# tj12323/GeoPurify

Measured on AMD Instinct MI355X. Metric: scenes/sec (ScanNet-val shape) + pooled-feature GB/s vs HBM peak, higher is better.
Workload: dtype f32 (student convolutions and pooling: f16 hi/lo split operands, 3 MFMAs per product, fp32 accumulate)

## Files before the change

### geopurify_amd/_lib.py

```python
import ctypes
import os
from ctypes import POINTER, c_char_p, c_double, c_float, c_int32, c_int64, c_size_t, c_uint32, c_uint64, c_void_p

_HERE = os.path.dirname(os.path.abspath(__file__))
LIB_PATH = os.environ.get("GP_LIB") or os.path.join(_HERE, "libgeopurify_hip.so")

_P = c_void_p
GP_KNN_MAX_K = 127
GP_KNN_QUERY_MAX_K = 32
GP_ELEM_F32, GP_ELEM_F16, GP_ELEM_BF16 = 0, 1, 2
GP_LABEL_U8, GP_LABEL_I16, GP_LABEL_I32, GP_LABEL_I64 = 0, 1, 2, 3

SIGNATURES = {
    "gp_version": (c_int32, []),
    "gp_last_error": (c_char_p, []),
    "gp_debug_set": (c_int32, [c_int32, c_int32]),
    "gp_debug_ptr": (c_int32, [c_int32, _P, c_size_t]),
    "gp_voxelize_workspace_bytes": (c_size_t, [c_int64]),
    "gp_voxelize_f64": (c_int32, [_P, c_int64, POINTER(c_double), _P, _P, _P, _P, _P, _P, _P, c_size_t, _P]),
    "gp_fnv_hash_f64": (c_int32, [_P, c_int64, _P, _P]),
    "gp_project_points_f64": (c_int32, [_P, c_int64, POINTER(c_double), c_double, c_double, c_double,
                                        c_double, _P, c_int32, c_int32, c_int32, c_double, _P, _P, _P]),
    "gp_render_depth_f64": (c_int32, [_P, c_int64, POINTER(c_double), c_double, c_double, c_double, c_double,
                                      c_int32, c_int32, c_int32, _P, _P]),
# ... 51 lines not shown
    "gp_pool_tiles_workspace_bytes": (c_size_t, [c_int64, c_int32]),
    "gp_pool_tiles_count": (c_int32, [_P, c_int64, c_int32, c_int32, _P, _P, c_size_t, _P]),
    "gp_pool_tiles_fill": (c_int32, [_P, _P, c_int64, c_int32, c_int32, _P, _P, _P, _P]),
    "gp_pool_tiles_apply": (c_int32, [_P, c_int64, _P, _P, _P, c_int32, c_int64, c_int32, _P, c_int64, _P]),
    "gp_pool_mfma_workspace_bytes": (c_size_t, [c_int64, c_int32]),
    "gp_pool_mfma_count": (c_int32, [_P, c_int64, c_int32, c_int32, c_int32, _P, _P, _P, c_size_t, _P]),
    "gp_pool_mfma_fill": (c_int32, [_P, _P, c_int64, c_int32, c_int32, _P, _P, c_int64, _P, _P, _P, _P]),
    "gp_pool_mfma_apply": (c_int32, [_P, _P, c_int64, _P, _P, _P, _P, c_int64, c_int32, c_int32, _P, _P, c_int64, _P, c_int64, _P, _P]),
    "gp_pool_mfma_apply_persistent": (c_int32, [_P, _P, c_int64, _P, _P, _P, _P, c_int64, c_int32, c_int32, c_int32, _P, _P, c_int64,
                                                _P, c_int64, c_int64, _P, _P, _P]),
    "gp_pool_cs_workspace_bytes": (c_size_t, [c_int64, c_int32]),
    "gp_pool_cs_count": (c_int32, [_P, c_int64, c_int32, c_int32, _P, _P, _P, _P, c_size_t, _P]),
    "gp_pool_cs_fill": (c_int32, [_P, _P, c_int64, c_int32, c_int32, _P, c_int64, c_int32, _P, _P, _P, _P, _P]),
    "gp_pool_cs_structure": (c_int32, [_P, c_int64, c_int32, c_int32, _P, c_int64, c_int32, _P, _P, _P, _P, _P, _P]),
    "gp_pool_cs_structure_valid": (c_int32, [_P, c_int64, c_int32, c_int32, _P, c_int64, c_int32, _P, _P, _P, _P]),
    "gp_affinity_cs_fragments": (c_int32, [_P, _P, c_int64, c_int32, c_int32, c_float, _P, _P, _P, _P, c_int32, _P, _P, _P]),
    "gp_pool_cs_apply": (c_int32, [_P, _P, c_int64, _P, _P, _P, _P, _P, c_int64, c_int32, c_int32, _P, _P, c_int64, _P, c_int64, _P, _P]),
    "gp_pool_cs_deps": (c_int32, [_P, _P, c_int64, c_int32, _P, _P, _P]),
    "gp_pool_cs_chain_flag_words": (c_size_t, [c_int64, c_int32]),
    "gp_pool_cs_chain_flag_words_d": (c_size_t, [c_int64, c_int32, c_int32]),
    "gp_pool_cs_apply_chain": (c_int32, [_P, _P, _P, _P, c_int64, _P, _P, _P, _P, _P, c_int64, c_int32, c_int32, c_int32, _P, c_int64, _P, _P, _P,
                                         c_uint32, _P]),
    "gp_lift_dense_accum": (c_int32, [_P, c_int32, c_int32, c_int32, _P, _P, _P, c_int64, _P, c_int64, _P, _P]),
    "gp_lift_dense_bilinear_accum": (c_int32, [_P, c_int32, c_int32, c_int32, c_int32, c_int32, _P, _P, _P, c_int64, _P,
                                               c_int64, _P, _P]),
    "gp_lift_dense_finish": (c_int32, [_P, c_int64, c_int32, _P, c_int64, _P, _P]),
    "gp_lift_masks_workspace_bytes": (c_size_t, [c_int32, c_int32, c_int32]),
    "gp_lift_masks_view": (c_int32, [_P, c_int32, c_int32, c_int32, _P, _P, _P, _P, _P, c_int32, c_int32,
                                     _P, _P, c_int64, _P, _P, _P, c_size_t, _P]),
    "gp_pv_count": (c_int32, [_P, c_int64, _P, _P]),
# ... 196 lines not shown
```

### geopurify_amd/csrc/pool_mfma_cs.hip

```cpp
#include <cstring>
#include <rocprim/device/device_scan.hpp>

#include "gp_common.h"
#include "gp_gfx950.h"
#include "gp_scan_bytes.h"


namespace {

constexpr int CS_KS = 32;
constexpr int CS_D = 512;
constexpr int CS_DMAX = 1024;
constexpr int CS_BR = 128;
constexpr int CS_NG = CS_BR / 16;
constexpr int CS_NC = 256;
constexpr int CS_NW = 8;
constexpr int CS_WC = CS_NC / CS_NW;
constexpr int CS_MAXID = 16384;
constexpr int CS_MAXNK = 12288;
constexpr int CS_HS = 16384;
constexpr float CS_WSCALE = GP_POOL_CS_WSCALE;

constexpr int CS_RB = CS_NC * 2;
constexpr int CS_PLANE = CS_KS * CS_RB;
// ... 11 lines not shown
}
__device__ __forceinline__ void cs_st_sc1(uint32_t *p, uint32_t v) {
    __hip_atomic_store(p, v, __ATOMIC_RELAXED, __HIP_MEMORY_SCOPE_AGENT);
}
template <typename V>
__device__ __forceinline__ void cs_st16_sc1(void *p, V v) {
    static_assert(sizeof(V) == 16, "16-byte store");
    asm volatile("global_store_dwordx4 %0, %1, off sc1\n\ts_nop 1" ::"v"(p), "v"(v) : "memory");
}

__device__ __forceinline__ void cs_wait_a(f16x8 (&h)[4], f16x8 (&l)[4]) {
    asm volatile("s_waitcnt lgkmcnt(0)"
                 : "+v"(h[0]), "+v"(h[1]), "+v"(h[2]), "+v"(h[3]), "+v"(l[0]), "+v"(l[1]), "+v"(l[2]), "+v"(l[3]));
}

__device__ int cs_union(const int32_t *__restrict__ nbr, int n, int *keys, int *dense, int cap) {
    __shared__ int s_wcnt[16];
    __shared__ int s_base, s_new, s_over;
    const int tid = threadIdx.x, lane = tid & 63, wv = tid >> 6;
    int hs = 2048, shift = 21;
    for (;;) {
        for (int i = tid; i < hs; i += 1024) keys[i] = -1;
        if (tid == 0) { s_base = 0; s_new = 0; s_over = 0; }
        __syncthreads();
        for (int i = tid; i < n; i += 1024) {
            const int id = nbr[i];
            unsigned h = ((unsigned)id * 2654435761u) >> shift;
            int probes = 0;
            while (true) {
                const int old = atomicCAS(&keys[h], -1, id);
                if (old == -1) { atomicAdd(&s_new, 1); break; }
                if (old == id) break;
                h = (h + 1) & (hs - 1);
                if (++probes > (hs < cap ? 256 : hs)) { s_over = 1; break; }
            }
        }
        __syncthreads();
        const bool over = s_over || (hs < cap && s_new > hs / 2);
        __syncthreads();
        if (!over) break;
        if (hs >= cap) return -1;
// ... 1 lines not shown
        shift = 32 - (31 - __clz(cap));
    }
    for (int i0 = 0; i0 < hs; i0 += 1024) {
        const int key = keys[i0 + tid];
        const unsigned long long m = __ballot(key >= 0);
        if (lane == 0) s_wcnt[wv] = __popcll(m);
        __syncthreads();
        int before = s_base;
        for (int w = 0; w < wv; ++w) before += s_wcnt[w];
        if (key >= 0) dense[before + __popcll(m & ((1ull << lane) - 1ull))] = key;
        __syncthreads();
        if (tid == 0) { int tot = 0; for (int w = 0; w < 16; ++w) tot += s_wcnt[w]; s_base += tot; }
        __syncthreads();
    }
    return s_base;
}

__global__ void __launch_bounds__(1024)
cs_count_kernel(const int32_t *__restrict__ nbr, int64_t nv, int k, int rpb, int64_t *__restrict__ padded_cnt, int32_t *__restrict__ bu_n,
                int cap, int second, unsigned long long *__restrict__ stats) {
    extern __shared__ int s_mem[];
    int *keys = s_mem, *dense = s_mem + cap;
    const int64_t b = blockIdx.x, r0 = b * rpb;
    if (second && bu_n[b] >= 0) return;
    const int rows = (int)((nv - r0) < rpb ? (nv - r0) : rpb);
    const int U = cs_union(nbr + r0 * k, rows * k, keys, dense, cap);
    if (threadIdx.x == 0) {
        padded_cnt[b] = U < 0 ? 0 : (int64_t)((U + CS_KS - 1) / CS_KS) * CS_KS;
        bu_n[b] = U;
        if (U > 0 && stats) atomicMax(stats, (unsigned long long)U);
    }
}

constexpr int CS_FILL_WEIGHTS = 0, CS_FILL_DST = 1, CS_FILL_VALID = 2;
template <int MODE>
__global__ void __launch_bounds__(1024)
cs_fill_kernel(const int32_t *__restrict__ nbr, const float *__restrict__ w, int64_t nv, int k, int rpb, const int64_t *__restrict__ bu_off,
               int32_t *__restrict__ bu_row, uint32_t *__restrict__ bu_mask, _Float16 *__restrict__ wa_hi, _Float16 *__restrict__ wa_lo,
               int32_t *__restrict__ dst, uint32_t *__restrict__ valid, int cap) {
    constexpr bool WEIGHTS = MODE == CS_FILL_WEIGHTS;
    extern __shared__ int s_mem[];
    int *A = s_mem, *B = s_mem + cap;
    unsigned short *npos = reinterpret_cast<unsigned short *>(s_mem + 2 * cap);
    const int tid = threadIdx.x;
    const int64_t b = blockIdx.x, r0 = b * rpb;
    const int rows = (int)((nv - r0) < rpb ? (nv - r0) : rpb);
    const int n = rows * k;
    const int32_t *nb = nbr + r0 * k;
    const int U = cs_union(nb, n, A, B, cap);
    int np2 = 1;
    while (np2 < U) np2 <<= 1;
    for (int i = U + tid; i < np2; i += 1024) B[i] = INT32_MAX;
    __syncthreads();
    gp_bitonic_sort_lds(B, np2, tid, 1024);
    for (int i = tid; i < U; i += 1024) A[i] = 0;
    __syncthreads();
    for (int t = tid; t < n; t += 1024) {
        const int id = nb[t];
        int lo = 0, hi = U - 1;
        while (lo < hi) { int mid = (lo + hi) >> 1; if (B[mid] < id) lo = mid + 1; else hi = mid; }
        atomicOr(&A[lo], 1 << ((t / k) >> 4));
    }
    __syncthreads();
    for (int i = tid; i < np2; i += 1024) {
        int key = INT32_MAX;
        if (i < U) {
            const int m = A[i];
            const int first = __ffs(m) - 1, last = 31 - __clz(m);
            key = (first << 28) | (last << 25) | (m << 14) | i;
        }
        A[i] = key;
    }
    __syncthreads();
    gp_bitonic_sort_lds(A, np2, tid, 1024);
    const int64_t o = bu_off[b];
    const int Up = (int)(bu_off[b + 1] - o);
    for (int p = tid; p < Up; p += 1024) {
        const int src = p < U ? (A[p] & 0x3FFF) : (A[0] & 0x3FFF);
        bu_row[o + p] = B[src];
        if (p < U) npos[src] = (unsigned short)p;
    }
    const int64_t ks0 = o / CS_KS;
    __shared__ unsigned s_mask[CS_MAXNK / CS_KS];
    for (int t = tid; t < Up / CS_KS; t += 1024) {
        unsigned m = 0;
        for (int p = t * CS_KS; p < (t + 1) * CS_KS && p < U; ++p) m |= (unsigned)(A[p] >> 14) & 0xFFu;
        bu_mask[ks0 + t] = m;
        s_mask[t] = m;
    }
    __syncthreads();
    if constexpr (MODE == CS_FILL_VALID) {
        const int nsteps = Up / CS_KS;
        const bool in_lds = nsteps * CS_BR <= cap;
        unsigned *sv = reinterpret_cast<unsigned *>(A);
        uint32_t *gv = valid + ks0 * CS_BR;
        __syncthreads();
        for (int i = tid; i < nsteps * CS_BR; i += 1024) { if (in_lds) sv[i] = 0u; else gv[i] = 0u; }
        __syncthreads();
        for (int t = tid; t < n; t += 1024) {
            const int rl = t / k;
            const int id = nb[t];
            int lo = 0, hi = U - 1;
            while (lo < hi) { int mid = (lo + hi) >> 1; if (B[mid] < id) lo = mid + 1; else hi = mid; }
            const int p = npos[lo];
            if (in_lds) atomicOr(&sv[(p / CS_KS) * CS_BR + rl], 1u << (p % CS_KS));
            else atomicOr(&gv[(p / CS_KS) * CS_BR + rl], 1u << (p % CS_KS));
        }
        if (in_lds) {
            __syncthreads();
            for (int i = tid; i < nsteps * CS_BR; i += 1024) gv[i] = sv[i];
        }
        return;
    }
    for (int i = tid; i < (Up / CS_KS) * CS_NG * 64; i += 1024) {
        const int f = i >> 6;
        if ((s_mask[f >> 3] >> (f & 7)) & 1u) {
            const f16x8 z = {0, 0, 0, 0, 0, 0, 0, 0};
            *reinterpret_cast<f16x8 *>(wa_hi + (ks0 * CS_NG * 64 + i) * 8) = z;
            *reinterpret_cast<f16x8 *>(wa_lo + (ks0 * CS_NG * 64 + i) * 8) = z;
        }
    }
    __syncthreads();
    for (int t = tid; t < n; t += 1024) {
        const int rl = t / k;
        const int id = nb[t];
        int lo = 0, hi = U - 1;
        while (lo < hi) { int mid = (lo + hi) >> 1; if (B[mid] < id) lo = mid + 1; else hi = mid; }
        const int p = npos[lo];
        const int64_t ks = ks0 + p / CS_KS;
        const int kk = p % CS_KS;
        const int64_t idx = ((ks * CS_NG + (rl >> 4)) * 64 + (kk >> 3) * 16 + (rl & 15)) * 8 + (kk & 7);
        if constexpr (WEIGHTS) {
            const float v = w[r0 * k + t] * GP_POOL_CS_WSCALE;
            gp_split_f16(v, wa_hi, wa_lo, idx);
        } else {
            dst[r0 * k + t] = (int32_t)idx;
        }
    }
}

struct CsChain {
    const _Float16 *a_hi, *a_lo;
    _Float16 *b_hi, *b_lo;
    int64_t ld;
    uint32_t *flags;
    const int32_t *dep;
    int32_t T;
    uint32_t base;
    int32_t half_sel = -1;
};
constexpr int CS_DEP_CAP = 64;
constexpr int CS_FLAG_HDR = 32;

// ... 738 lines not shown
extern "C" int gp_pool_cs_structure_valid(const int32_t *nbr, int64_t nv, int32_t k, int32_t rows_per_block, const int64_t *bu_off,
                                          int64_t total_rows, int32_t max_union, int32_t *bu_row, uint32_t *bu_mask, uint32_t *bu_valid,
                                          void *stream_) {
    GP_CHECK_ARG(nbr && bu_off && bu_row && bu_mask && bu_valid && nv > 0 && total_rows > 0 && total_rows % CS_KS == 0,
                 "gp_pool_cs_structure_valid: bad argument");
    GP_CHECK_ARG(cs_rpb_ok(rows_per_block), "gp_pool_cs_structure_valid: rows_per_block=%d (16..%d)", rows_per_block, CS_BR);
    GP_CHECK_ARG((int64_t)CS_BR * k <= CS_MAXNK, "gp_pool_cs_structure_valid: k=%d too large (128*k <= %d)", k, CS_MAXNK);
    int64_t nb = (nv + rows_per_block - 1) / rows_per_block;
    hipStream_t s = gp_stream(stream_);
    const size_t sm_max = (size_t)(CS_HS + CS_MAXID) * sizeof(int) + (size_t)CS_MAXNK * sizeof(unsigned short);
    const int cap = cs_fill_cap(max_union);
    GP_SMEM_ATTR(cs_fill_kernel<CS_FILL_VALID>, sm_max);
    GP_CHECK_HIP(hipMemsetAsync(bu_valid + total_rows / CS_KS * CS_BR, 0, 64 * sizeof(uint32_t), s));
    cs_fill_kernel<CS_FILL_VALID><<<(unsigned)nb, 1024, cs_fill_smem(cap, k), s>>>(nbr, nullptr, nv, k, rows_per_block, bu_off, bu_row, bu_mask, nullptr,
                                                                                  nullptr, nullptr, bu_valid, cap);
    GP_CHECK_LAUNCH();
    return GP_OK;
}

extern "C" int gp_affinity_cs_fragments(const void *e_hi, const void *e_lo, int64_t nv, int32_t d, int32_t k, float sharpen,
                                        const int64_t *bu_off, const int32_t *bu_row, const uint32_t *bu_mask, const uint32_t *bu_valid,
                                        int32_t rows_per_block, void *wa_hi, void *wa_lo, void *stream_) {
    GP_CHECK_ARG(e_hi && e_lo && bu_off && bu_row && bu_mask && bu_valid && wa_hi && wa_lo && nv > 0, "gp_affinity_cs_fragments: null/empty argument");
    GP_CHECK_ARG(d == AF_D, "gp_affinity_cs_fragments: d=%d (kernel specialised for %d-wide embeddings)", d, AF_D);
    GP_CHECK_ARG(k > 0 && k <= AF_KMAX, "gp_affinity_cs_fragments: k=%d (1..%d)", k, AF_KMAX);
    GP_CHECK_ARG(cs_rpb_ok(rows_per_block), "gp_affinity_cs_fragments: rows_per_block=%d (16..%d)", rows_per_block, CS_BR);
    GP_CHECK_ARG((uintptr_t)e_hi % 16 == 0 && (uintptr_t)e_lo % 16 == 0, "gp_affinity_cs_fragments: embedding planes must be 16-byte aligned");
    hipStream_t s = gp_stream(stream_);
    const int64_t nb = (nv + rows_per_block - 1) / rows_per_block;
    const int64_t per_xcd = (nb + 7) / 8;
// ... 93 lines not shown
```

### geopurify_amd/csrc/rcb.hip

```cpp
#include "gp_common.h"

namespace {

constexpr int RCB_MAX_SEG = 32;

template <int CH, int NT>
__global__ void __launch_bounds__(NT)
rcb_chunk_kernel(const int32_t *__restrict__ coords , int64_t nv, int leaf, int32_t *__restrict__ sigma, int32_t *__restrict__ rho) {
    __shared__ int s_c[3][CH];
    __shared__ unsigned s_key[CH];
    __shared__ unsigned short s_perm[2][CH];
    __shared__ unsigned char s_seg[CH];
    __shared__ int s_start[RCB_MAX_SEG + 1], s_len[RCB_MAX_SEG], s_axis[RCB_MAX_SEG], s_lo[RCB_MAX_SEG][3], s_hi[RCB_MAX_SEG][3];
    __shared__ int s_nseg, s_more;
    const int tid = threadIdx.x;
    const int64_t base = (int64_t)blockIdx.x * CH;
    const int n = (int)((nv - base) < CH ? (nv - base) : CH);
    for (int i = tid; i < CH; i += NT) {
        const int64_t r = base + (i < n ? i : n - 1);
        s_c[0][i] = coords[r * 3];
        s_c[1][i] = coords[r * 3 + 1];
        s_c[2][i] = coords[r * 3 + 2];
        s_perm[0][i] = (unsigned short)i;
    }
    if (tid == 0) { s_nseg = 1; s_start[0] = 0; s_len[0] = n; s_more = n > leaf; }
    __syncthreads();
    int cur = 0, level = 0;
    while (s_more) {
        const int nseg = s_nseg;
        for (int i = tid; i < nseg * 3; i += NT) { s_lo[i / 3][i % 3] = 0x7fffffff; s_hi[i / 3][i % 3] = -0x7fffffff; }
        for (int i = tid; i < CH; i += NT) {
            int sg = 0;
            if (i < n) {
                int lo = 0, hi = nseg - 1;
                while (lo < hi) { const int mid = (lo + hi + 1) >> 1; if (s_start[mid] <= i) lo = mid; else hi = mid - 1; }
                sg = lo;
            }
            s_seg[i] = (unsigned char)sg;
        }
        __syncthreads();
        for (int i = tid; i < n; i += NT) {
            const int sg = s_seg[i];
// ... 3 lines not shown
                for (int a = 0; a < 3; ++a) { atomicMin(&s_lo[sg][a], s_c[a][r]); atomicMax(&s_hi[sg][a], s_c[a][r]); }
            }
        }
        __syncthreads();
        if (tid < nseg) {
            int ax = 0, best = -1;
            if (s_len[tid] > leaf) {
#pragma unroll
                for (int a = 0; a < 3; ++a) { const int e = s_hi[tid][a] - s_lo[tid][a]; if (e > best) { best = e; ax = a; } }
            } else {
                ax = -1;
            }
            s_axis[tid] = ax;
        }
        __syncthreads();
        for (int i = tid; i < CH; i += NT) {
            unsigned k = 0xffffffffu;
            if (i < n) {
                const int sg = s_seg[i], ax = s_axis[sg];
                unsigned c = 0;
                if (ax >= 0) c = (unsigned)(s_c[ax][s_perm[cur][i]] - s_lo[sg][ax]) & 0x7fffu;
                k = ((unsigned)sg << 27) | (c << 12) | (unsigned)i;
            }
            s_key[i] = k;
        }
        __syncthreads();
        const int limit = (n == CH) ? (CH >> level) : CH;
        for (int kk = 2; kk <= limit; kk <<= 1)
            for (int j = kk >> 1; j > 0; j >>= 1) {
                for (int i = tid; i < CH; i += NT) {
                    const int ixj = i ^ j;
                    if (ixj > i) {
                        const unsigned x = s_key[i], y = s_key[ixj];
                        const bool up = (kk == limit) || ((i & kk) == 0);
                        if ((x > y) == up) { s_key[i] = y; s_key[ixj] = x; }
                    }
                }
                __syncthreads();
            }
        ++level;
        for (int i = tid; i < n; i += NT) s_perm[cur ^ 1][i] = s_perm[cur][s_key[i] & 0xfffu];
        cur ^= 1;
        if (tid == 0) {
            int ns = 0, more = 0;
            int st[RCB_MAX_SEG], ln[RCB_MAX_SEG];
            for (int sg = 0; sg < nseg; ++sg) {
                const int len = s_len[sg], start = s_start[sg];
                if (len > leaf && ns + 2 <= RCB_MAX_SEG) {
                    int half = ((len / 2 + leaf - 1) / leaf) * leaf;
                    if (half >= len) half = len / 2;
                    st[ns] = start; ln[ns] = half; ++ns;
                    st[ns] = start + half; ln[ns] = len - half; ++ns;
                    more |= (half > leaf) | (len - half > leaf);
                } else {
                    st[ns] = start; ln[ns] = len; ++ns;
                }
            }
// ... 19 lines not shown
        out[i] = rho[nbr[(int64_t)sigma[p] * k + j]];
    }
}

}

extern "C" int gp_rcb_order(const int32_t *coords, int64_t nv, int32_t chunk_rows, int32_t leaf_rows, int32_t *sigma, int32_t *rho,
                            void *stream_) {
    GP_CHECK_ARG(coords && sigma && rho && nv > 0, "gp_rcb_order: null/empty argument");
    GP_CHECK_ARG(chunk_rows == 1024 || chunk_rows == 2048, "gp_rcb_order: chunk_rows=%d (1024 or 2048: a chunk lives in one workgroup's LDS)", chunk_rows);
    GP_CHECK_ARG(leaf_rows >= 16 && chunk_rows % leaf_rows == 0 && chunk_rows / leaf_rows <= RCB_MAX_SEG,
                 "gp_rcb_order: leaf_rows=%d must divide the chunk into at most %d leaves", leaf_rows, RCB_MAX_SEG);
    GP_CHECK_ARG(nv < ((int64_t)1 << 31), "gp_rcb_order: row ids are 32-bit");
    hipStream_t s = gp_stream(stream_);
    const unsigned blocks = (unsigned)((nv + chunk_rows - 1) / chunk_rows);
    if (chunk_rows == 1024) rcb_chunk_kernel<1024, 256><<<blocks, 256, 0, s>>>(coords, nv, leaf_rows, sigma, rho);
    else rcb_chunk_kernel<2048, 512><<<blocks, 512, 0, s>>>(coords, nv, leaf_rows, sigma, rho);
    GP_CHECK_LAUNCH();
    return GP_OK;
}

extern "C" int gp_rows_renumber_i32(const int32_t *nbr, int64_t nv, int32_t k, const int32_t *sigma, const int32_t *rho, int32_t *out,
                                    void *stream_) {
    GP_CHECK_ARG(nbr && sigma && rho && out && nv > 0 && k > 0 && out != nbr, "gp_rows_renumber_i32: null/empty argument (out must not alias nbr)");
    rows_renumber_kernel<<<2048, 256, 0, gp_stream(stream_)>>>(nbr, nv, k, sigma, rho, out);
    GP_CHECK_LAUNCH();
    return GP_OK;
}
```

### geopurify_amd/ops.py

```python
import ctypes

import numpy as np
import torch

from . import _lib
from ._lib import check


def _ptr(t):
    return ctypes.c_void_p(t.data_ptr()) if t is not None else None


def _stream():
    return ctypes.c_void_p(torch.cuda.current_stream().cuda_stream)


def _ws(nbytes, device):
    return torch.empty(max(int(nbytes), 256), dtype=torch.uint8, device=device)


def _chk(t, dtype, name):
    if t.dtype != dtype or not t.is_cuda or not t.is_contiguous():
        raise ValueError(f"{name}: expected contiguous CUDA {dtype}, got {t.dtype} cuda={t.is_cuda} contig={t.is_contiguous()}")
    return t
# ... 759 lines not shown
    assert xh.stride(0) == xl.stride(0)
    yh, yl = out_split if out_split is not None else (None, None)
    check(lib.gp_pool_mfma_apply(_ptr(xh), _ptr(xl), xh.stride(0), _ptr(op.bu_off), _ptr(op.bu_row), _ptr(op.wa_hi),
                                 _ptr(op.wa_lo), op.nv, int(d), int(op.block_rows), _ptr(yh), _ptr(yl),
                                 yh.stride(0) if yh is not None else 0, _ptr(out_f32),
                                 out_f32.stride(0) if out_f32 is not None else 0, _ptr(out_scale), _stream()), "gp_pool_mfma_apply")
    return out_f32 if out_f32 is not None else out_split


class PoolCs:

    def __init__(self, bu_off, bu_n, bu_row, bu_mask, wa_hi, wa_lo, nv, total, block_rows=128):
        self.bu_off, self.bu_n, self.bu_row, self.bu_mask = bu_off, bu_n, bu_row, bu_mask
        self.wa_hi, self.wa_lo, self.nv, self.total = wa_hi, wa_lo, nv, total
        self.block_rows = block_rows
        self.dst = None
        self.max_union = 0
        self.valid = None
        self.k = 0
        self.dep = self.flags = None
        self.epoch = 0
        self.filled = False


def pool_cs_plan(nbr, rows_per_block=128, structure=False):
    lib = _lib.load()
    nv, k = nbr.shape
    dev = nbr.device
    rpb = int(rows_per_block)
    nb = (nv + rpb - 1) // rpb
    ws = _ws(lib.gp_pool_cs_workspace_bytes(nv, rpb), dev)
    bu_off = torch.empty(nb + 2, dtype=torch.int64, device=dev)[:nb + 1]
    bu_n = torch.empty(nb, dtype=torch.int32, device=dev)
    tail = bu_off.as_strided((2,), (1,), bu_off.storage_offset() + nb)
    check(lib.gp_pool_cs_count(_ptr(nbr), nv, int(k), rpb, _ptr(bu_off), _ptr(bu_n), tail[1:].data_ptr(), _ptr(ws), ws.numel(), _stream()),
          "gp_pool_cs_count")
    total, max_union = (int(v) for v in readback(tail))
    bu_row = torch.empty(total, dtype=torch.int32, device=dev)
    bu_mask = torch.empty(total // 32, dtype=torch.int32, device=dev)
    wa_hi = torch.empty(total // 32 * 8 * 512, dtype=torch.float16, device=dev)
    wa_lo = torch.empty_like(wa_hi)
    op = PoolCs(bu_off, bu_n, bu_row, bu_mask, wa_hi, wa_lo, nv, total, block_rows=rpb)
    op.max_union = max_union
    if structure == "valid":
        op.valid = torch.empty(total // 32 * 128 + 64, dtype=torch.int32, device=dev)
        check(lib.gp_pool_cs_structure_valid(_ptr(nbr), nv, int(k), rpb, _ptr(bu_off), total, max_union, _ptr(bu_row), _ptr(bu_mask),
                                             _ptr(op.valid), _stream()), "gp_pool_cs_structure_valid")
        op.k = int(k)
        return op
    if structure and total * 128 < 2 ** 31:
        op.dst = torch.empty((nv, k), dtype=torch.int32, device=dev)
        check(lib.gp_pool_cs_structure(_ptr(nbr), nv, int(k), rpb, _ptr(bu_off), total, max_union, _ptr(bu_row), _ptr(bu_mask), _ptr(wa_hi),
                                       _ptr(wa_lo), _ptr(op.dst), _stream()), "gp_pool_cs_structure")
    return op


def pool_cs_fill(op, nbr, w):
    lib = _lib.load()
    nv, k = nbr.shape
    check(lib.gp_pool_cs_fill(_ptr(nbr), _ptr(w), nv, int(k), int(op.block_rows), _ptr(op.bu_off), op.total, int(op.max_union), _ptr(op.bu_row),
                              _ptr(op.bu_mask), _ptr(op.wa_hi), _ptr(op.wa_lo), _stream()), "gp_pool_cs_fill")
    op.filled = True
# ... 1761 lines not shown
```

### geopurify_amd/pipeline.py

```python
from dataclasses import dataclass, field
from typing import List, Optional

import numpy as np
import torch

from . import ops
from .bicubic import aa_bicubic_taps

GEO_DIM = 6
CONV_PAD = 32


def _pad_to(v, m):
    return (v + m - 1) // m * m


class StudentWeights:

    def __init__(self, state_dict, device, eps=1e-5, mode="f16x3", residual_from_planes=True, interleaved_rows=True, blocked_weights=True,
                 head="f16x3"):
        sd = {k: v.detach() for k, v in state_dict.items()}
        self.mode = mode
        self.residual_from_planes = bool(residual_from_planes)
        self.interleaved_rows = bool(interleaved_rows)
# ... 487 lines not shown
        else:
            grid = ops.grid_build(cs)
        nbr_map = ops.kernel_map_build(grid, cs)
        pairs = ops.conv_pairs_build(nbr_map, col_tiles=max(1, st.hidden // 256)) if any(l[0] == "f16x3" for l in st.layers) else None
        mark("grid+kernel_map")
        nbr = ops.knn_lattice(grid, cs, perm, self.K)
        mark("kNN")
        state = {"X": X, "rank": rank, "nbr_map": nbr_map, "pairs": pairs, "nbr": nbr, "Nv": Nv, "D": D, "pool": None,
                 "xs": xs if xs is not None else st.split_input(X)}
        if family in ("cs", "chain"):
            if sc is None:
                sc = ops.pow2_scale(X, D)
            how = self.pool_structure_ahead
            if how and self.affinity_mfma and self.K <= 96 and self.student is not None and self.student.embed == 128:
                how = "valid"
            rho = None
            nbr_op = nbr
            if how == "valid" and self.pool_row_order == "rcb" and Nv > 1024:
                sigma, rho = ops.rcb_order(cs, 1024, 128)
                nbr_op = ops.rows_renumber(nbr, sigma, rho)
                state["rank_pool"] = rho[rank.long()].contiguous()
            state["pool"] = {"op": ops.pool_cs_plan(nbr_op, structure=how), "sc": sc, "rho": rho, "nbr": nbr_op,
                             "x_split": ops.split_f16(X, D, scale=sc[0:1], dst_row=rho),
                             "pong": tuple(torch.empty((Nv, D), dtype=torch.float16, device=dev) for _ in range(2))}
            if family == "chain" and (state["pool"]["op"].dst is not None or state["pool"]["op"].valid is not None):
                ops.pool_cs_deps(state["pool"]["op"], D)
            mark("pool plan+split")
        return state

    def refine(self, batch: SceneBatch, F, after_student=None, prepared=None, classify_text=None):
        p = prepared if prepared is not None else self.prepare(batch, F)
        X, rank, nbr, Nv, D = p["X"], p["rank"], p["nbr"], p["Nv"], p["D"]
        mark = self.stage_mark if self.stage_mark is not None else (lambda name: None)
        op = p["pool"]["op"] if p["pool"] is not None else None
        mfma_aff = op is not None and op.valid is not None
        rho = p["pool"]["rho"] if (p["pool"] is not None and mfma_aff) else None
        E = self.student.forward(X, p["nbr_map"], p["pairs"], x_split=p.get("xs"), mark=self.stage_mark, planes=mfma_aff, plane_rows=rho)
# ... 183 lines not shown
```

### include/geopurify_hip.h

```cpp
#ifndef GEOPURIFY_HIP_H
#define GEOPURIFY_HIP_H

#include <stddef.h>
#include <stdint.h>

#ifdef __cplusplus
extern "C" {
#endif

#define GP_OK 0
#define GP_EINVAL (-22)
#define GP_ENOMEM (-12)
#define GP_EHIP (-5)
#define GP_ERANGE (-34)

#define GP_KNN_MAX_K 127

#define GP_ELEM_F32 0
#define GP_ELEM_F16 1
#define GP_ELEM_BF16 2

int gp_version(void);
int gp_debug_set(int32_t key, int32_t value);
int gp_debug_ptr(int32_t key, void *device_buffer, size_t bytes);
// ... 146 lines not shown
                                  int32_t d, int32_t block_rows, int32_t min_steps, void *y_hi, void *y_lo,
                                  int64_t ld_y, float *y_f32, int64_t ld_yf, int64_t y_rows,
                                  const float *out_scale, uint32_t *queue, void *stream);

size_t gp_pool_cs_workspace_bytes(int64_t nv, int32_t rows_per_block);
int gp_pool_cs_count(const int32_t *nbr, int64_t nv, int32_t k, int32_t rows_per_block, int64_t *bu_off, int32_t *bu_n,
                     int64_t *max_union, void *workspace, size_t workspace_bytes, void *stream);
int gp_pool_cs_fill(const int32_t *nbr, const float *w, int64_t nv, int32_t k, int32_t rows_per_block, const int64_t *bu_off,
                    int64_t total_rows, int32_t max_union, int32_t *bu_row, uint32_t *bu_mask, void *wa_hi, void *wa_lo, void *stream);
int gp_pool_cs_structure(const int32_t *nbr, int64_t nv, int32_t k, int32_t rows_per_block, const int64_t *bu_off,
                         int64_t total_rows, int32_t max_union, int32_t *bu_row, uint32_t *bu_mask, void *wa_hi, void *wa_lo,
                         int32_t *dst, void *stream);
int gp_pool_cs_structure_valid(const int32_t *nbr, int64_t nv, int32_t k, int32_t rows_per_block, const int64_t *bu_off,
                               int64_t total_rows, int32_t max_union, int32_t *bu_row, uint32_t *bu_mask, uint32_t *bu_valid,
                               void *stream);
int gp_affinity_cs_fragments(const void *e_hi, const void *e_lo, int64_t nv, int32_t d, int32_t k, float sharpen,
                             const int64_t *bu_off, const int32_t *bu_row, const uint32_t *bu_mask, const uint32_t *bu_valid,
                             int32_t rows_per_block, void *wa_hi, void *wa_lo, void *stream);
int gp_pool_cs_apply(const void *x_hi, const void *x_lo, int64_t ld_x, const int64_t *bu_off, const int32_t *bu_row,
                     const uint32_t *bu_mask, const void *wa_hi, const void *wa_lo, int64_t nv, int32_t d,
                     int32_t rows_per_block, void *y_hi, void *y_lo, int64_t ld_y, float *y_f32, int64_t ld_yf,
                     const float *out_scale, void *stream);
int gp_pool_cs_deps(const int64_t *bu_off, const int32_t *bu_row, int64_t nv, int32_t rows_per_block, int32_t *dep,
                    int32_t *scratch, void *stream);
size_t gp_pool_cs_chain_flag_words(int64_t nv, int32_t rows_per_block);
size_t gp_pool_cs_chain_flag_words_d(int64_t nv, int32_t rows_per_block, int32_t d);
int gp_pool_cs_apply_chain(void *x_hi, void *x_lo, void *p_hi, void *p_lo, int64_t ld, const int64_t *bu_off,
                           const int32_t *bu_row, const uint32_t *bu_mask, const void *wa_hi, const void *wa_lo, int64_t nv,
                           int32_t d, int32_t rows_per_block, int32_t applications, float *y_f32, int64_t ld_yf,
                           const float *out_scale, const int32_t *dep, uint32_t *flags, uint32_t epoch, void *stream);
// ... 346 lines not shown
```

Before: 46.35.

## Fuse row renumbering into pool union count and cache sorted unions for structure pass

The pool planning count kernel now optionally applies the RCB row permutation inline, writes renumbered neighbours, and stores each block's sorted union ids in a workspace. A new structure-valid kernel reuses those stored ids instead of recomputing the hash union and bitonic sort. Small sorts are replaced with rank-by-count, neighbour ids are held in registers to avoid repeated binary searches, and the RCB kernel uses 1024 threads with a counting placement instead of bitonic passes. This trades extra workspace and a second fallback count launch for fewer planning kernels and less redundant sorting.

```diff
diff --git a/geopurify_amd/_lib.py b/geopurify_amd/_lib.py
--- a/geopurify_amd/_lib.py
+++ b/geopurify_amd/_lib.py
@@ -89,6 +89,10 @@
     "gp_pool_cs_fill": (c_int32, [_P, _P, c_int64, c_int32, c_int32, _P, c_int64, c_int32, _P, _P, _P, _P, _P]),
     "gp_pool_cs_structure": (c_int32, [_P, c_int64, c_int32, c_int32, _P, c_int64, c_int32, _P, _P, _P, _P, _P, _P]),
     "gp_pool_cs_structure_valid": (c_int32, [_P, c_int64, c_int32, c_int32, _P, c_int64, c_int32, _P, _P, _P, _P]),
+    "gp_pool_cs_union_slot": (c_int64, [c_int64, c_int32, c_int32]),
+    "gp_pool_cs_sorted_workspace_bytes": (c_size_t, [c_int64, c_int32, c_int32]),
+    "gp_pool_cs_count_sorted": (c_int32, [_P, c_int64, c_int32, c_int32, _P, _P, _P, _P, _P, _P, _P, c_size_t, _P]),
+    "gp_pool_cs_structure_valid_sorted": (c_int32, [_P, c_int64, c_int32, c_int32, _P, _P, _P, c_size_t, c_int64, c_int32, _P, _P, _P, _P]),
     "gp_affinity_cs_fragments": (c_int32, [_P, _P, c_int64, c_int32, c_int32, c_float, _P, _P, _P, _P, c_int32, _P, _P, _P]),
     "gp_pool_cs_apply": (c_int32, [_P, _P, c_int64, _P, _P, _P, _P, _P, c_int64, c_int32, c_int32, _P, _P, c_int64, _P, c_int64, _P, _P]),
     "gp_pool_cs_deps": (c_int32, [_P, _P, c_int64, c_int32, _P, _P, _P]),
diff --git a/geopurify_amd/csrc/pool_mfma_cs.hip b/geopurify_amd/csrc/pool_mfma_cs.hip
--- a/geopurify_amd/csrc/pool_mfma_cs.hip
+++ b/geopurify_amd/csrc/pool_mfma_cs.hip
@@ -49,7 +49,16 @@
                  : "+v"(h[0]), "+v"(h[1]), "+v"(h[2]), "+v"(h[3]), "+v"(l[0]), "+v"(l[1]), "+v"(l[2]), "+v"(l[3]));
 }
 
-__device__ int cs_union(const int32_t *__restrict__ nbr, int n, int *keys, int *dense, int cap) {
+constexpr int CS_TRIPS = CS_MAXNK / 1024;
+__device__ __forceinline__ void cs_load_ids(const int32_t *__restrict__ nb, int n, int (&idv)[CS_TRIPS]) {
+#pragma unroll
+    for (int t = 0; t < CS_TRIPS; ++t) {
+        const int i = (int)threadIdx.x + 1024 * t;
+        idv[t] = i < n ? nb[i] : -1;
+    }
+}
+
+__device__ __forceinline__ int cs_union_ids(const int (&idv)[CS_TRIPS], int *keys, int *dense, int cap) {
     __shared__ int s_wcnt[16];
     __shared__ int s_base, s_new, s_over;
     const int tid = threadIdx.x, lane = tid & 63, wv = tid >> 6;
@@ -58,8 +67,10 @@
         for (int i = tid; i < hs; i += 1024) keys[i] = -1;
         if (tid == 0) { s_base = 0; s_new = 0; s_over = 0; }
         __syncthreads();
-        for (int i = tid; i < n; i += 1024) {
-            const int id = nbr[i];
+#pragma unroll
+        for (int t = 0; t < CS_TRIPS; ++t) {
+            const int id = idv[t];
+            if (id < 0) continue;
             unsigned h = ((unsigned)id * 2654435761u) >> shift;
             int probes = 0;
             while (true) {
@@ -91,6 +102,26 @@
         __syncthreads();
     }
     return s_base;
+}
+__device__ __forceinline__ int cs_union(const int32_t *__restrict__ nbr, int n, int *keys, int *dense, int cap) {
+    int idv[CS_TRIPS];
+    cs_load_ids(nbr, n, idv);
+    return cs_union_ids(idv, keys, dense, cap);
+}
+
+__device__ __forceinline__ void cs_rank_by_count(const int *v, int U, int np2, int *rank) {
+    const int tid = threadIdx.x;
+    if (tid < U) rank[tid] = 0;
+    __syncthreads();
+    const int parts = 1024 / np2, e = tid & (np2 - 1), part = tid / np2;
+    if (e < U) {
+        const int per = (U + parts - 1) / parts, j0 = part * per, j1 = min(U, j0 + per);
+        const int mine = v[e];
+        int c = 0;
+        for (int j = j0; j < j1; ++j) c += v[j] < mine;
+        if (c) atomicAdd(&rank[e], c);
+    }
+    __syncthreads();
 }
 
 __global__ void __launch_bounds__(1024)
@@ -109,7 +140,67 @@
     }
 }
 
+template <bool RENUM>
+__global__ void __launch_bounds__(1024)
+cs_count_sorted_kernel(const int32_t *__restrict__ nbr, int64_t nv, int k, int rpb, const int32_t *__restrict__ sigma,
+                       const int32_t *__restrict__ rho, int32_t *__restrict__ nbr_out, int64_t *__restrict__ padded_cnt,
+                       int32_t *__restrict__ bu_n, int32_t *__restrict__ ids, int64_t slot, int cap, int second,
+                       unsigned long long *__restrict__ stats) {
+    extern __shared__ int s_mem[];
+    int *keys = s_mem, *dense = s_mem + cap;
+    const int tid = threadIdx.x;
+    const int64_t b = blockIdx.x, r0 = b * rpb;
+    if (second && bu_n[b] >= 0) return;
+    const int rows = (int)((nv - r0) < rpb ? (nv - r0) : rpb);
+    const int n = rows * k;
+    int idv[CS_TRIPS];
+    if constexpr (RENUM) {
+        int32_t *ob = nbr_out + r0 * k;
+        int col[CS_TRIPS];
+#pragma unroll
+        for (int t = 0; t < CS_TRIPS; ++t) {
+            const int i = tid + 1024 * t, rl = i / k;
+            col[t] = i - rl * k;
+            idv[t] = i < n ? sigma[r0 + rl] : 0;
+        }
+#pragma unroll
+        for (int t = 0; t < CS_TRIPS; ++t) idv[t] = tid + 1024 * t < n ? nbr[(int64_t)idv[t] * k + col[t]] : 0;
+#pragma unroll
+        for (int t = 0; t < CS_TRIPS; ++t) idv[t] = tid + 1024 * t < n ? rho[idv[t]] : -1;
+#pragma unroll
+        for (int t = 0; t < CS_TRIPS; ++t)
+            if (tid + 1024 * t < n) ob[tid + 1024 * t] = idv[t];
+    } else {
+        cs_load_ids(nbr + r0 * k, n, idv);
+    }
+    const int U = cs_union_ids(idv, keys, dense, cap);
+    if (tid == 0) {
+        padded_cnt[b] = U < 0 ? 0 : (int64_t)((U + CS_KS - 1) / CS_KS) * CS_KS;
+        bu_n[b] = U;
+        if (U > 0 && stats) atomicMax(stats, (unsigned long long)U);
+    }
+    if (U < 0) return;
+    int np2 = 1;
+    while (np2 < U) np2 <<= 1;
+    int32_t *out = ids + b * slot;
+    if (np2 <= 1024) {
+        cs_rank_by_count(dense, U, np2, keys);
+        if (tid < U && keys[tid] < slot) out[keys[tid]] = dense[tid];
+        return;
+    }
+    for (int i = U + tid; i < np2; i += 1024) dense[i] = INT32_MAX;
+    __syncthreads();
+    gp_bitonic_sort_lds(dense, np2, tid, 1024);
+    for (int i = tid; i < U && i < slot; i += 1024) out[i] = dense[i];
+}
+
 constexpr int CS_FILL_WEIGHTS = 0, CS_FILL_DST = 1, CS_FILL_VALID = 2;
+template <int MODE>
+__device__ __forceinline__ void
+cs_fill_sorted(const int32_t *__restrict__ nb, const float *__restrict__ w, int k, int64_t b, int64_t r0, int n, int U, int np2, int *A, int *B,
+               unsigned short *npos, unsigned *sv, int sv_cap, const int64_t *__restrict__ bu_off, int32_t *__restrict__ bu_row,
+               uint32_t *__restrict__ bu_mask, _Float16 *__restrict__ wa_hi, _Float16 *__restrict__ wa_lo, int32_t *__restrict__ dst,
+               uint32_t *__restrict__ valid);
 template <int MODE>
 __global__ void __launch_bounds__(1024)
 cs_fill_kernel(const int32_t *__restrict__ nbr, const float *__restrict__ w, int64_t nv, int k, int rpb, const int64_t *__restrict__ bu_off,
@@ -130,13 +221,30 @@
     for (int i = U + tid; i < np2; i += 1024) B[i] = INT32_MAX;
     __syncthreads();
     gp_bitonic_sort_lds(B, np2, tid, 1024);
+    cs_fill_sorted<MODE>(nb, w, k, b, r0, n, U, np2, A, B, npos, reinterpret_cast<unsigned *>(A), cap, bu_off, bu_row, bu_mask, wa_hi, wa_lo,
+                         dst, valid);
+}
+
+template <int MODE>
+__device__ __forceinline__ void
+cs_fill_sorted(const int32_t *__restrict__ nb, const float *__restrict__ w, int k, int64_t b, int64_t r0, int n, int U, int np2, int *A, int *B,
+               unsigned short *npos, unsigned *sv, int sv_cap, const int64_t *__restrict__ bu_off, int32_t *__restrict__ bu_row,
+               uint32_t *__restrict__ bu_mask, _Float16 *__restrict__ wa_hi, _Float16 *__restrict__ wa_lo, int32_t *__restrict__ dst,
+               uint32_t *__restrict__ valid) {
+    constexpr bool WEIGHTS = MODE == CS_FILL_WEIGHTS;
+    const int tid = threadIdx.x;
+    int pos[CS_TRIPS];
+    cs_load_ids(nb, n, pos);
     for (int i = tid; i < U; i += 1024) A[i] = 0;
     __syncthreads();
-    for (int t = tid; t < n; t += 1024) {
-        const int id = nb[t];
+#pragma unroll
+    for (int t = 0; t < CS_TRIPS; ++t) {
+        const int id = pos[t];
+        if (id < 0) continue;
         int lo = 0, hi = U - 1;
         while (lo < hi) { int mid = (lo + hi) >> 1; if (B[mid] < id) lo = mid + 1; else hi = mid; }
-        atomicOr(&A[lo], 1 << ((t / k) >> 4));
+        pos[t] = lo;
+        atomicOr(&A[lo], 1 << (((tid + 1024 * t) / k) >> 4));
     }
     __syncthreads();
     for (int i = tid; i < np2; i += 1024) {
@@ -149,7 +257,16 @@
         A[i] = key;
     }
     __syncthreads();
-    gp_bitonic_sort_lds(A, np2, tid, 1024);
+    if (np2 <= 1024) {
+        int *rank = A + np2;
+        cs_rank_by_count(A, U, np2, rank);
+        const int key = tid < U ? A[tid] : 0, r = tid < U ? rank[tid] : 0;
+        __syncthreads();
+        if (tid < U) A[r] = key;
+        __syncthreads();
+    } else {
+        gp_bitonic_sort_lds(A, np2, tid, 1024);
+    }
     const int64_t o = bu_off[b];
     const int Up = (int)(bu_off[b + 1] - o);
     for (int p = tid; p < Up; p += 1024) {
@@ -168,18 +285,16 @@
     __syncthreads();
     if constexpr (MODE == CS_FILL_VALID) {
         const int nsteps = Up / CS_KS;
-        const bool in_lds = nsteps * CS_BR <= cap;
-        unsigned *sv = reinterpret_cast<unsigned *>(A);
+        const bool in_lds = nsteps * CS_BR <= sv_cap;
         uint32_t *gv = valid + ks0 * CS_BR;
         __syncthreads();
         for (int i = tid; i < nsteps * CS_BR; i += 1024) { if (in_lds) sv[i] = 0u; else gv[i] = 0u; }
         __syncthreads();
-        for (int t = tid; t < n; t += 1024) {
-            const int rl = t / k;
-            const int id = nb[t];
-            int lo = 0, hi = U - 1;
-            while (lo < hi) { int mid = (lo + hi) >> 1; if (B[mid] < id) lo = mid + 1; else hi = mid; }
-            const int p = npos[lo];
+#pragma unroll
+        for (int t = 0; t < CS_TRIPS; ++t) {
+            if (pos[t] < 0) continue;
+            const int rl = (tid + 1024 * t) / k;
+            const int p = npos[pos[t]];
             if (in_lds) atomicOr(&sv[(p / CS_KS) * CS_BR + rl], 1u << (p % CS_KS));
             else atomicOr(&gv[(p / CS_KS) * CS_BR + rl], 1u << (p % CS_KS));
         }
@@ -198,12 +313,12 @@
         }
     }
     __syncthreads();
-    for (int t = tid; t < n; t += 1024) {
+#pragma unroll
+    for (int i = 0; i < CS_TRIPS; ++i) {
+        if (pos[i] < 0) continue;
+        const int t = tid + 1024 * i;
         const int rl = t / k;
-        const int id = nb[t];
-        int lo = 0, hi = U - 1;
-        while (lo < hi) { int mid = (lo + hi) >> 1; if (B[mid] < id) lo = mid + 1; else hi = mid; }
-        const int p = npos[lo];
+        const int p = npos[pos[i]];
         const int64_t ks = ks0 + p / CS_KS;
         const int kk = p % CS_KS;
         const int64_t idx = ((ks * CS_NG + (rl >> 4)) * 64 + (kk >> 3) * 16 + (rl & 15)) * 8 + (kk & 7);
@@ -214,6 +329,29 @@
             dst[r0 * k + t] = (int32_t)idx;
         }
     }
+}
+
+__global__ void __launch_bounds__(1024)
+cs_structure_sorted_kernel(const int32_t *__restrict__ nbr, int64_t nv, int k, int rpb, const int64_t *__restrict__ bu_off,
+                           const int32_t *__restrict__ bu_n, const int32_t *__restrict__ ids, int64_t slot, int32_t *__restrict__ bu_row,
+                           uint32_t *__restrict__ bu_mask, uint32_t *__restrict__ valid, int cap, int sv_words) {
+    extern __shared__ int s_mem[];
+    int *A = s_mem, *B = s_mem + cap;
+    unsigned short *npos = reinterpret_cast<unsigned short *>(s_mem + 2 * cap);
+    unsigned *sv = reinterpret_cast<unsigned *>(s_mem + 2 * cap + CS_BR * k / 2);
+    const int tid = threadIdx.x;
+    const int64_t b = blockIdx.x, r0 = b * rpb;
+    const int rows = (int)((nv - r0) < rpb ? (nv - r0) : rpb);
+    const int n = rows * k;
+    int U = bu_n[b];
+    if (U < 1 || U > cap || U > slot || U > n) return;
+    const int32_t *src = ids + b * slot;
+    int np2 = 1;
+    while (np2 < U) np2 <<= 1;
+    for (int i = tid; i < U; i += 1024) B[i] = src[i];
+    __syncthreads();
+    cs_fill_sorted<CS_FILL_VALID>(nbr + r0 * k, nullptr, k, b, r0, n, U, np2, A, B, npos, sv_words ? sv : reinterpret_cast<unsigned *>(A),
+                                  sv_words ? sv_words : cap, bu_off, bu_row, bu_mask, nullptr, nullptr, nullptr, valid);
 }
 
 struct CsChain {
@@ -982,6 +1120,88 @@
     GP_CHECK_HIP(hipMemsetAsync(bu_valid + total_rows / CS_KS * CS_BR, 0, 64 * sizeof(uint32_t), s));
     cs_fill_kernel<CS_FILL_VALID><<<(unsigned)nb, 1024, cs_fill_smem(cap, k), s>>>(nbr, nullptr, nv, k, rows_per_block, bu_off, bu_row, bu_mask, nullptr,
                                                                                   nullptr, nullptr, bu_valid, cap);
+    GP_CHECK_LAUNCH();
+    return GP_OK;
+}
+
+static int64_t cs_union_slot(int64_t nv, int32_t k, int32_t rpb) {
+    const int64_t per_block = (int64_t)rpb * k;
+    return per_block < nv ? per_block : nv;
+}
+extern "C" int64_t gp_pool_cs_union_slot(int64_t nv, int32_t k, int32_t rows_per_block) {
+    if (nv <= 0 || k <= 0 || !cs_rpb_ok(rows_per_block) || (int64_t)CS_BR * k > CS_MAXNK) return 0;
+    return cs_union_slot(nv, k, rows_per_block);
+}
+extern "C" size_t gp_pool_cs_sorted_workspace_bytes(int64_t nv, int32_t k, int32_t rows_per_block) {
+    if (nv <= 0 || k <= 0 || !cs_rpb_ok(rows_per_block) || (int64_t)CS_BR * k > CS_MAXNK) return 0;
+    int64_t nb = (nv + rows_per_block - 1) / rows_per_block;
+    GpCarver cv(nullptr, 0);
+    cv.take<int64_t>(nb + 1);
+    cv.take<char>(gp_scan_bytes<int64_t>(nb + 1));
+    cv.take<int32_t>((size_t)nb * (size_t)cs_union_slot(nv, k, rows_per_block));
+    return cv.off;
+}
+
+extern "C" int gp_pool_cs_count_sorted(const int32_t *nbr, int64_t nv, int32_t k, int32_t rows_per_block, const int32_t *sigma,
+                                       const int32_t *rho, int32_t *nbr_out, int64_t *bu_off, int32_t *bu_n, int64_t *max_union,
+                                       void *workspace, size_t workspace_bytes, void *stream_) {
+    GP_CHECK_ARG(nbr && bu_off && bu_n && workspace && nv > 0 && k > 0, "gp_pool_cs_count_sorted: null/empty argument");
+    GP_CHECK_ARG(cs_rpb_ok(rows_per_block), "gp_pool_cs_count_sorted: rows_per_block=%d (16..%d)", rows_per_block, CS_BR);
+    GP_CHECK_ARG((int64_t)CS_BR * k <= CS_MAXNK, "gp_pool_cs_count_sorted: k=%d too large (128*k <= %d)", k, CS_MAXNK);
+    GP_CHECK_ARG((sigma != nullptr) == (rho != nullptr) && (sigma != nullptr) == (nbr_out != nullptr) && nbr_out != nbr,
+                 "gp_pool_cs_count_sorted: sigma, rho and nbr_out come together (nbr_out must not alias nbr)");
+    GP_CHECK_ARG(nv < ((int64_t)1 << 31), "gp_pool_cs_count_sorted: row ids are 32-bit");
+    int64_t nb = (nv + rows_per_block - 1) / rows_per_block;
+    const int64_t slot = cs_union_slot(nv, k, rows_per_block);
+    GpCarver cv(workspace, workspace_bytes);
+    int64_t *cnt = cv.take<int64_t>(nb + 1);
+    size_t tb = gp_scan_bytes<int64_t>(nb + 1);
+    char *tmp = cv.take<char>(tb);
+    int32_t *ids = cv.take<int32_t>((size_t)nb * (size_t)slot);
+    if (!cv.ok()) { gp_set_error("gp_pool_cs_count_sorted: workspace too small"); return GP_ENOMEM; }
+    hipStream_t s = gp_stream(stream_);
+    GP_CHECK_HIP(hipMemsetAsync(cnt + nb, 0, sizeof(int64_t), s));
+    if (max_union) GP_CHECK_HIP(hipMemsetAsync(max_union, 0, sizeof(int64_t), s));
+    const int cap_big = CS_HS > cs_np2((int64_t)CS_BR * k) ? CS_HS : cs_np2((int64_t)CS_BR * k);
+    unsigned long long *stats = reinterpret_cast<unsigned long long *>(max_union);
+    GP_SMEM_ATTR(cs_count_sorted_kernel<false>, (size_t)2 * CS_HS * sizeof(int));
+    if (sigma)
+        cs_count_sorted_kernel<true><<<(unsigned)nb, 1024, (size_t)2 * 2048 * sizeof(int), s>>>(nbr, nv, k, rows_per_block, sigma, rho, nbr_out, cnt,
+                                                                                               bu_n, ids, slot, 2048, 0, stats);
+    else
+        cs_count_sorted_kernel<false><<<(unsigned)nb, 1024, (size_t)2 * 2048 * sizeof(int), s>>>(nbr, nv, k, rows_per_block, nullptr, nullptr, nullptr,
+                                                                                                cnt, bu_n, ids, slot, 2048, 0, stats);
+    cs_count_sorted_kernel<false><<<(unsigned)nb, 1024, (size_t)2 * cap_big * sizeof(int), s>>>(sigma ? nbr_out : nbr, nv, k, rows_per_block, nullptr,
+                                                                                               nullptr, nullptr, cnt, bu_n, ids, slot, cap_big, 1, stats);
+    GP_CHECK_HIP(rocprim::exclusive_scan(tmp, tb, cnt, bu_off, (int64_t)0, (size_t)(nb + 1), rocprim::plus<int64_t>(), s));
+    GP_CHECK_LAUNCH();
+    return GP_OK;
+}
+
+extern "C" int gp_pool_cs_structure_valid_sorted(const int32_t *nbr, int64_t nv, int32_t k, int32_t rows_per_block, const int64_t *bu_off,
+                                                 const int32_t *bu_n, const void *workspace, size_t workspace_bytes, int64_t total_rows,
+                                                 int32_t max_union, int32_t *bu_row, uint32_t *bu_mask, uint32_t *bu_valid, void *stream_) {
+    GP_CHECK_ARG(nbr && bu_off && bu_n && workspace && bu_row && bu_mask && bu_valid && nv > 0 && k > 0 && total_rows > 0 &&
+                     total_rows % CS_KS == 0 && max_union > 0,
+                 "gp_pool_cs_structure_valid_sorted: bad argument");
+    GP_CHECK_ARG(cs_rpb_ok(rows_per_block), "gp_pool_cs_structure_valid_sorted: rows_per_block=%d (16..%d)", rows_per_block, CS_BR);
+    GP_CHECK_ARG((int64_t)CS_BR * k <= CS_MAXNK, "gp_pool_cs_structure_valid_sorted: k=%d too large (128*k <= %d)", k, CS_MAXNK);
+    int64_t nb = (nv + rows_per_block - 1) / rows_per_block;
+    const int64_t slot = cs_union_slot(nv, k, rows_per_block);
+    GpCarver cv(const_cast<void *>(workspace), workspace_bytes);
+    cv.take<int64_t>(nb + 1);
+    cv.take<char>(gp_scan_bytes<int64_t>(nb + 1));
+    const int32_t *ids = cv.take<int32_t>((size_t)nb * (size_t)slot);
+    if (!cv.ok()) { gp_set_error("gp_pool_cs_structure_valid_sorted: workspace too small"); return GP_ENOMEM; }
+    hipStream_t s = gp_stream(stream_);
+    const int cap = cs_fill_cap(max_union);
+    const int64_t sv_need = ((int64_t)max_union + CS_KS - 1) / CS_KS * CS_BR;
+    const int sv_words = sv_need * (int64_t)sizeof(uint32_t) <= 32768 ? (int)sv_need : 0;
+    const size_t sm_max = (size_t)(CS_HS + CS_MAXID) * sizeof(int) + (size_t)CS_MAXNK * sizeof(unsigned short);
+    GP_SMEM_ATTR(cs_structure_sorted_kernel, sm_max);
+    GP_CHECK_HIP(hipMemsetAsync(bu_valid + total_rows / CS_KS * CS_BR, 0, 64 * sizeof(uint32_t), s));
+    cs_structure_sorted_kernel<<<(unsigned)nb, 1024, cs_fill_smem(cap, k) + (size_t)sv_words * sizeof(uint32_t), s>>>(
+        nbr, nv, k, rows_per_block, bu_off, bu_n, ids, slot, bu_row, bu_mask, bu_valid, cap, sv_words);
     GP_CHECK_LAUNCH();
     return GP_OK;
 }
diff --git a/geopurify_amd/csrc/rcb.hip b/geopurify_amd/csrc/rcb.hip
--- a/geopurify_amd/csrc/rcb.hip
+++ b/geopurify_amd/csrc/rcb.hip
@@ -25,7 +25,7 @@
     }
     if (tid == 0) { s_nseg = 1; s_start[0] = 0; s_len[0] = n; s_more = n > leaf; }
     __syncthreads();
-    int cur = 0, level = 0;
+    int cur = 0;
     while (s_more) {
         const int nseg = s_nseg;
         for (int i = tid; i < nseg * 3; i += NT) { s_lo[i / 3][i % 3] = 0x7fffffff; s_hi[i / 3][i % 3] = -0x7fffffff; }
@@ -59,33 +59,25 @@
             s_axis[tid] = ax;
         }
         __syncthreads();
-        for (int i = tid; i < CH; i += NT) {
-            unsigned k = 0xffffffffu;
-            if (i < n) {
-                const int sg = s_seg[i], ax = s_axis[sg];
-                unsigned c = 0;
-                if (ax >= 0) c = (unsigned)(s_c[ax][s_perm[cur][i]] - s_lo[sg][ax]) & 0x7fffu;
-                k = ((unsigned)sg << 27) | (c << 12) | (unsigned)i;
-            }
-            s_key[i] = k;
+        for (int i = tid; i < n; i += NT) {
+            const int sg = s_seg[i], ax = s_axis[sg];
+            if (ax >= 0) s_key[i] = (((unsigned)(s_c[ax][s_perm[cur][i]] - s_lo[sg][ax]) & 0x7fffu) << 12) | (unsigned)i;
         }
         __syncthreads();
-        const int limit = (n == CH) ? (CH >> level) : CH;
-        for (int kk = 2; kk <= limit; kk <<= 1)
-            for (int j = kk >> 1; j > 0; j >>= 1) {
-                for (int i = tid; i < CH; i += NT) {
-                    const int ixj = i ^ j;
-                    if (ixj > i) {
-                        const unsigned x = s_key[i], y = s_key[ixj];
-                        const bool up = (kk == limit) || ((i & kk) == 0);
-                        if ((x > y) == up) { s_key[i] = y; s_key[ixj] = x; }
-                    }
-                }
-                __syncthreads();
+        for (int i = tid; i < n; i += NT) {
+            const int sg = s_seg[i];
+            int to = i;
+            if (s_axis[sg] >= 0) {
+                const unsigned mine = s_key[i];
+                const int j0 = s_start[sg], j1 = j0 + s_len[sg];
+                int c = 0;
+                for (int j = j0; j < j1; ++j) c += s_key[j] < mine;
+                to = j0 + c;
             }
-        ++level;
-        for (int i = tid; i < n; i += NT) s_perm[cur ^ 1][i] = s_perm[cur][s_key[i] & 0xfffu];
+            s_perm[cur ^ 1][to] = s_perm[cur][i];
+        }
         cur ^= 1;
+        __syncthreads();
         if (tid == 0) {
             int ns = 0, more = 0;
             int st[RCB_MAX_SEG], ln[RCB_MAX_SEG];
@@ -135,8 +127,8 @@
     GP_CHECK_ARG(nv < ((int64_t)1 << 31), "gp_rcb_order: row ids are 32-bit");
     hipStream_t s = gp_stream(stream_);
     const unsigned blocks = (unsigned)((nv + chunk_rows - 1) / chunk_rows);
-    if (chunk_rows == 1024) rcb_chunk_kernel<1024, 256><<<blocks, 256, 0, s>>>(coords, nv, leaf_rows, sigma, rho);
-    else rcb_chunk_kernel<2048, 512><<<blocks, 512, 0, s>>>(coords, nv, leaf_rows, sigma, rho);
+    if (chunk_rows == 1024) rcb_chunk_kernel<1024, 1024><<<blocks, 1024, 0, s>>>(coords, nv, leaf_rows, sigma, rho);
+    else rcb_chunk_kernel<2048, 1024><<<blocks, 1024, 0, s>>>(coords, nv, leaf_rows, sigma, rho);
     GP_CHECK_LAUNCH();
     return GP_OK;
 }
diff --git a/geopurify_amd/ops.py b/geopurify_amd/ops.py
--- a/geopurify_amd/ops.py
+++ b/geopurify_amd/ops.py
@@ -797,6 +797,7 @@
         self.bu_off, self.bu_n, self.bu_row, self.bu_mask = bu_off, bu_n, bu_row, bu_mask
         self.wa_hi, self.wa_lo, self.nv, self.total = wa_hi, wa_lo, nv, total
         self.block_rows = block_rows
+        self.nbr = None
         self.dst = None
         self.max_union = 0
         self.valid = None
@@ -806,18 +807,32 @@
         self.filled = False
 
 
-def pool_cs_plan(nbr, rows_per_block=128, structure=False):
+def pool_cs_plan(nbr, rows_per_block=128, structure=False, order=None, one_pass=True):
     lib = _lib.load()
     nv, k = nbr.shape
     dev = nbr.device
     rpb = int(rows_per_block)
     nb = (nv + rpb - 1) // rpb
-    ws = _ws(lib.gp_pool_cs_workspace_bytes(nv, rpb), dev)
+    if order is not None and structure != "valid":
+        raise ValueError("pool_cs_plan: a row order comes with structure='valid'")
+    one_pass = bool(one_pass) and structure == "valid"
     bu_off = torch.empty(nb + 2, dtype=torch.int64, device=dev)[:nb + 1]
     bu_n = torch.empty(nb, dtype=torch.int32, device=dev)
     tail = bu_off.as_strided((2,), (1,), bu_off.storage_offset() + nb)
-    check(lib.gp_pool_cs_count(_ptr(nbr), nv, int(k), rpb, _ptr(bu_off), _ptr(bu_n), tail[1:].data_ptr(), _ptr(ws), ws.numel(), _stream()),
-          "gp_pool_cs_count")
+    if one_pass:
+        ws = _ws(lib.gp_pool_cs_sorted_workspace_bytes(nv, int(k), rpb), dev)
+        sigma, rho = order if order is not None else (None, None)
+        nbr_out = torch.empty_like(nbr) if order is not None else None
+        check(lib.gp_pool_cs_count_sorted(_ptr(nbr), nv, int(k), rpb, _ptr(sigma), _ptr(rho), _ptr(nbr_out), _ptr(bu_off), _ptr(bu_n),
+                                          tail[1:].data_ptr(), _ptr(ws), ws.numel(), _stream()), "gp_pool_cs_count_sorted")
+        if nbr_out is not None:
+            nbr = nbr_out
+    else:
+        if order is not None:
+            nbr = rows_renumber(nbr, *order)
+        ws = _ws(lib.gp_pool_cs_workspace_bytes(nv, rpb), dev)
+        check(lib.gp_pool_cs_count(_ptr(nbr), nv, int(k), rpb, _ptr(bu_off), _ptr(bu_n), tail[1:].data_ptr(), _ptr(ws), ws.numel(), _stream()),
+              "gp_pool_cs_count")
     total, max_union = (int(v) for v in readback(tail))
     bu_row = torch.empty(total, dtype=torch.int32, device=dev)
     bu_mask = torch.empty(total // 32, dtype=torch.int32, device=dev)
@@ -825,10 +840,16 @@
     wa_lo = torch.empty_like(wa_hi)
     op = PoolCs(bu_off, bu_n, bu_row, bu_mask, wa_hi, wa_lo, nv, total, block_rows=rpb)
     op.max_union = max_union
+    op.nbr = nbr
     if structure == "valid":
         op.valid = torch.empty(total // 32 * 128 + 64, dtype=torch.int32, device=dev)
-        check(lib.gp_pool_cs_structure_valid(_ptr(nbr), nv, int(k), rpb, _ptr(bu_off), total, max_union, _ptr(bu_row), _ptr(bu_mask),
-                                             _ptr(op.valid), _stream()), "gp_pool_cs_structure_valid")
+        if one_pass:
+            check(lib.gp_pool_cs_structure_valid_sorted(_ptr(nbr), nv, int(k), rpb, _ptr(bu_off), _ptr(bu_n), _ptr(ws), ws.numel(), total,
+                                                        max_union, _ptr(bu_row), _ptr(bu_mask), _ptr(op.valid), _stream()),
+                  "gp_pool_cs_structure_valid_sorted")
+        else:
+            check(lib.gp_pool_cs_structure_valid(_ptr(nbr), nv, int(k), rpb, _ptr(bu_off), total, max_union, _ptr(bu_row), _ptr(bu_mask),
+                                                 _ptr(op.valid), _stream()), "gp_pool_cs_structure_valid")
         op.k = int(k)
         return op
     if structure and total * 128 < 2 ** 31:
diff --git a/geopurify_amd/pipeline.py b/geopurify_amd/pipeline.py
--- a/geopurify_amd/pipeline.py
+++ b/geopurify_amd/pipeline.py
@@ -525,13 +525,13 @@
             how = self.pool_structure_ahead
             if how and self.affinity_mfma and self.K <= 96 and self.student is not None and self.student.embed == 128:
                 how = "valid"
-            rho = None
-            nbr_op = nbr
+            rho = order = None
             if how == "valid" and self.pool_row_order == "rcb" and Nv > 1024:
-                sigma, rho = ops.rcb_order(cs, 1024, 128)
-                nbr_op = ops.rows_renumber(nbr, sigma, rho)
+                order = ops.rcb_order(cs, 1024, 128)
+                rho = order[1]
                 state["rank_pool"] = rho[rank.long()].contiguous()
-            state["pool"] = {"op": ops.pool_cs_plan(nbr_op, structure=how), "sc": sc, "rho": rho, "nbr": nbr_op,
+            op = ops.pool_cs_plan(nbr, structure=how, order=order)
+            state["pool"] = {"op": op, "sc": sc, "rho": rho, "nbr": op.nbr,
                              "x_split": ops.split_f16(X, D, scale=sc[0:1], dst_row=rho),
                              "pong": tuple(torch.empty((Nv, D), dtype=torch.float16, device=dev) for _ in range(2))}
             if family == "chain" and (state["pool"]["op"].dst is not None or state["pool"]["op"].valid is not None):
diff --git a/include/geopurify_hip.h b/include/geopurify_hip.h
--- a/include/geopurify_hip.h
+++ b/include/geopurify_hip.h
@@ -184,6 +184,14 @@
 int gp_pool_cs_structure_valid(const int32_t *nbr, int64_t nv, int32_t k, int32_t rows_per_block, const int64_t *bu_off,
                                int64_t total_rows, int32_t max_union, int32_t *bu_row, uint32_t *bu_mask, uint32_t *bu_valid,
                                void *stream);
+int64_t gp_pool_cs_union_slot(int64_t nv, int32_t k, int32_t rows_per_block);
+size_t gp_pool_cs_sorted_workspace_bytes(int64_t nv, int32_t k, int32_t rows_per_block);
+int gp_pool_cs_count_sorted(const int32_t *nbr, int64_t nv, int32_t k, int32_t rows_per_block, const int32_t *sigma, const int32_t *rho,
+                            int32_t *nbr_out, int64_t *bu_off, int32_t *bu_n, int64_t *max_union, void *workspace,
+                            size_t workspace_bytes, void *stream);
+int gp_pool_cs_structure_valid_sorted(const int32_t *nbr, int64_t nv, int32_t k, int32_t rows_per_block, const int64_t *bu_off,
+                                      const int32_t *bu_n, const void *workspace, size_t workspace_bytes, int64_t total_rows,
+                                      int32_t max_union, int32_t *bu_row, uint32_t *bu_mask, uint32_t *bu_valid, void *stream);
 int gp_affinity_cs_fragments(const void *e_hi, const void *e_lo, int64_t nv, int32_t d, int32_t k, float sharpen,
                              const int64_t *bu_off, const int32_t *bu_row, const uint32_t *bu_mask, const uint32_t *bu_valid,
                              int32_t rows_per_block, void *wa_hi, void *wa_lo, void *stream);
```

After: 46.73, median of 6. No clear change (+0.8%).
